# lenskit/csr

Measured on AMD Instinct MI355X. Metric: spmv_gflops, higher is better.
Workload: dtype f64

## Files before the change

### csr_amd/csrc/acc_groups.h

```cpp
#pragma once
#include <algorithm>
#include <cstdint>
#include <numeric>
#include <vector>

namespace csrk {
namespace accgroups {

constexpr int MAX_GROUPS = 3;
constexpr int XCDS = 8;

struct Deal {
    std::vector<std::vector<int32_t>> groups;
    std::vector<int32_t> first;
};

inline Deal deal_rows(const int64_t *lens, int32_t n, int G, int32_t cap)
{
    Deal d;
    d.first.push_back(0);
    if (n <= 0) return d;
    if (cap < 1) cap = 1;
    if (G < 1) G = 1;
    if (G > MAX_GROUPS) G = MAX_GROUPS;
// ... 24 lines not shown
}

constexpr int64_t TILE_ENTRIES = 512;
constexpr int64_t MIN_SEG_TILES = 48;
inline int choose_groups(const int64_t *lens, int32_t n, int g_max, int32_t cap, int64_t floor_len, int64_t nb, int32_t cus)
{
    if (cap < 1) cap = 1;
    if (g_max > MAX_GROUPS) g_max = MAX_GROUPS;
    if (g_max < 2 || n <= cap) return 1;
    std::vector<int64_t> sl;
    for (int32_t i = 0; i < n; i++)
        if (lens[i] >= floor_len) sl.push_back(lens[i]);
    for (int g = g_max; g > 1; g--) {
        const int64_t k = std::min<int64_t>((int64_t)sl.size(), (int64_t)g * cap);
        if (k <= (int64_t)(g - 1) * cap) continue;
        if (k < (int64_t)sl.size()) std::nth_element(sl.begin(), sl.begin() + k, sl.end(), [](int64_t a, int64_t b) { return a > b; });
        int64_t entries = 0;
        for (int64_t i = 0; i < k; i++) entries += sl[(size_t)i];
        if (entries / TILE_ENTRIES >= MIN_SEG_TILES * ((int64_t)g * nb + cus)) return g;
    }
    return 1;
}

inline int32_t group_wgs(int32_t cus, int gb, int g)
{
    const int32_t n = cus / gb + (g < cus % gb ? 1 : 0);
    return n < 1 ? 1 : n;
}

inline std::vector<uint32_t> place_wgs(const int32_t *n_wg, int gb)
{
    int64_t total = 0;
    int32_t w_max = 0;
    for (int g = 0; g < gb; g++) {
        total += n_wg[g];
        w_max = std::max(w_max, n_wg[g]);
    }
    std::vector<uint32_t> map((size_t)total, ~0u);
    int64_t fill[XCDS], room[XCDS];
    for (int c = 0; c < XCDS; c++) {
        fill[c] = 0;
        room[c] = total / XCDS + (c < total % XCDS ? 1 : 0);
    }
    std::vector<uint32_t> late;
    for (int32_t w = 0; w < w_max; w++)
        for (int g = 0; g < gb; g++) {
// ... 17 lines not shown
```

### csr_amd/csrc/fix56.h

```cpp
#pragma once
#include <cstdint>
#include <cstring>

#if defined(__HIPCC__)
#define FIX56_HD __host__ __device__ __forceinline__
#else
#define FIX56_HD inline
#endif

namespace csrk {
namespace fix56 {

constexpr int TILE = 512;
constexpr int LO_BYTES = TILE * 4, MID_BYTES = TILE * 2, HI_BYTES = TILE;
constexpr int MID_OFF = LO_BYTES, HI_OFF = LO_BYTES + MID_BYTES;
constexpr int TILE_BYTES = LO_BYTES + MID_BYTES + HI_BYTES;
constexpr uint64_t MANT_MASK = (1ull << 52) - 1;
constexpr uint32_t W_MANT = 0x000fffffu, W_SIGN = 0x00800000u;

struct Packed {
    unsigned char b[7];
};
static_assert(sizeof(Packed) * TILE == TILE_BYTES, "a tile of Packed entries is the three planes");

// ... 69 lines not shown
FIX56_HD double decode(uint32_t lo, uint32_t w, uint32_t ebits, double magic)
{
    const double d = double_of((w & W_MANT) | ebits, lo) - magic;
    return double_of((uint32_t)(bits_of(d) >> 32) ^ ((w & W_SIGN) << 8), (uint32_t)bits_of(d));
}
FIX56_HD uint32_t ebits_of(int32_t g) { return (uint32_t)(1075 + g) << 20; }
FIX56_HD double magic_of(int32_t g) { return double_of(ebits_of(g), 0u); }

FIX56_HD int lo_slot(int e) { return ((e & 7) >> 2) * 256 + (e >> 3) * 4 + (e & 3); }

FIX56_HD void put(unsigned char *tile, int e, uint64_t p)
{
    ((uint32_t *)tile)[lo_slot(e)] = lo_of(p);
    ((uint16_t *)(tile + MID_OFF))[e] = mid_of(p);
    tile[HI_OFF + e] = hi_of(p);
}
FIX56_HD double get(const unsigned char *tile, int e, int32_t g)
{
    const uint32_t lo = ((const uint32_t *)tile)[lo_slot(e)];
    const uint32_t w = (uint32_t)((const uint16_t *)(tile + MID_OFF))[e] | (uint32_t)tile[HI_OFF + e] << 16;
    return decode(lo, w, ebits_of(g), magic_of(g));
}

}
}
```

### csr_amd/csrc/spmv.hip

```cpp
#include "spmv_plan.h"

#include <algorithm>
#include <ctime>

namespace csrk {
template <bool R32>
__device__ __forceinline__ double spmv_prod(double a, double x)
{
    const double t = a * x;
    return R32 ? (double)(float)t : t;
}

void free_spmv_plan(SpmvPlan *p) { delete p; }

void spmv_plan_bytes_by_part(const SpmvPlan *p, int64_t out[5])
{
    for (int i = 0; i < 5; i++) out[i] = 0;
    auto add = [&](int part, std::initializer_list<const DevBuf *> bufs) {
        for (const DevBuf *b : bufs) out[part] += (int64_t)b->bytes;
    };
    for (const AccPanel *ap : p->acc) add(0, {&ap->row_list, &ap->vals, &ap->idx, &ap->tile_row0, &ap->segs, &ap->wg_seg, &ap->partial, &ap->z, &ap->wg_map});
    const Panel &t = p->tier1;
    add(1, {&t.row_list, &t.rp, &t.ci, &t.vs, &t.tile, &t.group, &t.carry_row, &t.carry_val, &t.y, &t.crp, &t.cidx});
    const LightStream *l = &p->ls;
// ... 462 lines not shown
                        v[u] = *((const F64x2 *)(x + w0) + tid + u * PT);
                    } else {
                        const f32x2_t t = *((const F32x2 *)(x + w0) + tid + u * PT);
                        v[u].x = (double)t.x;
                        v[u].y = (double)t.y;
                    }
                }
#pragma unroll
                for (int u = 0; u < WL; u++) ((f64x2_t *)s_x)[tid + u * PT] = v[u];
            } else {
                for (int k = tid; k < wlen; k += PT) s_x[k] = (double)x[w0 + k];
            }
        }
        __syncthreads();

        const int nt = sg.ntiles;
        AccVals<SV> v, vn;
        u32x4_t ix, ixn;
        int32_t tr0 = 0, tr0n = 0;
        int t = wv;
        const int64_t pstep = (int64_t)A.n_wg;
        if (t < nt) {
            const u32x4_t *ip = (const u32x4_t *)(pidx + (sg.ptile0 + t * pstep) * ACC_TILE);
            v.load(pvals + (sg.ptile0 + t * pstep) * ACC_TILE, lane);
            ix = __builtin_nontemporal_load(ip + lane);
            tr0 = tile_row0[sg.tile0 + t];
        }
        for (; t < nt; t += NW) {
            const bool more = t + NW < nt;
            if (more) {
                const u32x4_t *ip = (const u32x4_t *)(pidx + (sg.ptile0 + (t + NW) * pstep) * ACC_TILE);
                vn.load(pvals + (sg.ptile0 + (t + NW) * pstep) * ACC_TILE, lane);
                ixn = __builtin_nontemporal_load(ip + lane);
                tr0n = tile_row0[sg.tile0 + t + NW];
            }
            const uint32_t e[ACC_K] = {ix.x & 0xffffu, ix.x >> 16, ix.y & 0xffffu, ix.y >> 16,
                                       ix.z & 0xffffu, ix.z >> 16, ix.w & 0xffffu, ix.w >> 16};
            double a[ACC_K];
            v.get(a, fx_g);
            double xv[ACC_K];
#pragma unroll
            for (int j = 0; j < ACC_K; j++) xv[j] = s_x[e[j] & ACC_COL_MASK];
            int rw[ACC_K];
            {
                int lsum = 0;
#pragma unroll
                for (int j = 0; j < ACC_K; j++) lsum += (int)(e[j] >> ACC_ROW_SHIFT);
                int run = tr0 + wave_exscan_i32(lsum, lane);
#pragma unroll
                for (int j = 0; j < ACC_K; j++) {
                    run += (int)(e[j] >> ACC_ROW_SHIFT);
                    rw[j] = run;
                }
            }
            const int hr = rw[0];
            int cur = hr;
            double acc = 0.0, hs = 0.0;
            bool nb = false;
#pragma unroll
            for (int j = 0; j < ACC_K; j++) {
                const int r = rw[j];
                if (r != cur) {
// ... 535 lines not shown
{
    for (const void *f : {(const void *)spmv_acc_kernel<ACC_CB, ACC_THREADS>, (const void *)spmv_lstream_kernel<LS_PLAIN>,
                          (const void *)spmv_lstream_kernel<LS_RND>, (const void *)spmv_lstream_kernel<LS_PLAIN, true>,
                          (const void *)spmv_lstream_kernel<LS_RND, true>, (const void *)spmv_acc_kernel<ACC_CB, ACC_THREADS, true>,
                          (const void *)spmv_lstream_kernel<LS_PLAIN, false, true>, (const void *)spmv_lstream_kernel<LS_RND, false, true>,
                          (const void *)spmv_lstream_kernel<LS_PLAIN, true, true>, (const void *)spmv_lstream_kernel<LS_RND, true, true>,
                          (const void *)spmv_acc_kernel<ACC_CB, ACC_THREADS, false, float>,
                          (const void *)spmv_acc_kernel<ACC_CB, ACC_THREADS, true, float>,
                          (const void *)spmv_lstream_kernel<LS_PLAIN, false, false, float>, (const void *)spmv_lstream_kernel<LS_RND, false, false, float>,
                          (const void *)spmv_lstream_kernel<LS_PLAIN, true, false, float>, (const void *)spmv_lstream_kernel<LS_RND, true, false, float>,
                          (const void *)spmv_lstream_kernel<LS_PLAIN, false, true, float>, (const void *)spmv_lstream_kernel<LS_RND, false, true, float>,
                          (const void *)spmv_lstream_kernel<LS_PLAIN, true, true, float>, (const void *)spmv_lstream_kernel<LS_RND, true, true, float>,
                          (const void *)spmv_lstream_kernel<LS_RND24>, (const void *)spmv_lstream_kernel<LS_RND24, true>,
                          (const void *)spmv_lstream_kernel<LS_RND24, false, true>, (const void *)spmv_lstream_kernel<LS_RND24, true, true>,
                          (const void *)spmv_lstream_kernel<LS_RND24, false, false, float>, (const void *)spmv_lstream_kernel<LS_RND24, true, false, float>,
                          (const void *)spmv_lstream_kernel<LS_RND24, false, true, float>, (const void *)spmv_lstream_kernel<LS_RND24, true, true, float>,
                          (const void *)spmv_acc_kernel<ACC_CB, ACC_THREADS, false, double, float>,
                          (const void *)spmv_acc_kernel<ACC_CB, ACC_THREADS, true, double, float>,
                          (const void *)spmv_acc_kernel<ACC_CB, ACC_THREADS, false, float, float>,
                          (const void *)spmv_acc_kernel<ACC_CB, ACC_THREADS, true, float, float>,
                          (const void *)spmv_acc_kernel<ACC_CB, ACC_THREADS, false, fix56::Packed>,
                          (const void *)spmv_acc_kernel<ACC_CB, ACC_THREADS, true, fix56::Packed>,
                          (const void *)spmv_acc_kernel<ACC_CB, ACC_THREADS, false, fix56::Packed, float>,
                          (const void *)spmv_acc_kernel<ACC_CB, ACC_THREADS, true, fix56::Packed, float>})
        CSRK_HIP(hipFuncSetAttribute(f, hipFuncAttributeMaxDynamicSharedMemorySize, (int)(160 * 1024)));
    CSRK_HIP(hipFuncSetAttribute((const void *)ls_stage_kernel<double>, hipFuncAttributeMaxDynamicSharedMemorySize, (int)(LS_STAGE_WMAX * 8)));
    CSRK_HIP(hipFuncSetAttribute((const void *)ls_stage_kernel<float>, hipFuncAttributeMaxDynamicSharedMemorySize, (int)(LS_STAGE_WMAX * 8)));
    return CSRK_OK;
}

static int get_plan_locked(Matrix *m, hipStream_t s, SpmvPlan **out, bool launching)
{
    if (launching) m->spmv_calls++;
    const char *env = getenv("CSRK_SPMV_HEAVY_SPLIT"), *env_hot = getenv("CSRK_SPMV_HOT"), *env_ls = getenv("CSRK_SPMV_STREAM");
    const bool eager = (env && env[0] == '1') || (env_hot && env_hot[0] == '1') || (env_ls && env_ls[0] == '1') || !launching;
    const bool want_split = eager || m->spmv_calls >= 2;
    if (m->spmv_plan && !m->spmv_plan->split_considered && want_split && m->spmv_plan->algo == CSRK_SPMV_MERGE &&
        !m->spmv_plan->profiling) {
        if (hipDeviceSynchronize() != hipSuccess) {
            set_error("device synchronisation failed: %s", hipGetErrorString(hipGetLastError()));
            return CSRK_ERR_HIP;
        }
        free_spmv_plan(m->spmv_plan);
        m->spmv_plan = nullptr;
    }
    if (!m->spmv_plan) {
        SpmvPlan *p = new (std::nothrow) SpmvPlan();
// ... 92 lines not shown
        }
        bool t0_rides = false;
        if (do_heavy && p->n_heavy && !p->acc.empty()) {
            KernelTimer kh(p, s, 1);
            for (size_t a0 = 0; a0 < p->acc.size(); a0 += (size_t)p->acc[a0]->launch_groups) {
                AccPanel *ap = p->acc[a0];
                const int gb = ap->launch_groups;
                if (gb < 1 || gb > accgroups::MAX_GROUPS || a0 + (size_t)gb > p->acc.size()) {
                    set_error("internal: tier 0's groups and launches disagree");
                    return CSRK_ERR_INVALID;
                }
                AccLaunchArgs L = {};
                size_t lds = 0;
                for (int g = 0; g < gb; g++) {
                    const AccPanel *aq = p->acc[a0 + (size_t)g];
                    L.g[g] = {aq->vals.p, aq->idx.as<uint16_t>(), aq->tile_row0.as<int32_t>(), aq->segs.as<AccSeg>(),
                              aq->wg_seg.as<int32_t>(), aq->partial.as<double>(), aq->nrow, aq->n_wg, aq->fx_g, 0};
                    lds = aq->lds > lds ? aq->lds : lds;
                }
                L.wg_map = gb > 1 ? ap->wg_map.as<uint32_t>() : nullptr;
                const unsigned n_blocks = (unsigned)(gb > 1 ? ap->launch_wgs : ap->n_wg);
#define ACC_LAUNCH(SV) spmv_acc_kernel<ACC_CB, ACC_THREADS, R32, SV, XT><<<n_blocks, ACC_THREADS, lds, s>>>(L, d_x, m->ncols)
                if (ap->f32) ACC_LAUNCH(float);
                else if (ap->fix56) ACC_LAUNCH(fix56::Packed);
                else ACC_LAUNCH(double);
#undef ACC_LAUNCH
                CSRK_LAUNCH_CHECK();
            }
            kh.stop();
        }
        if (do_heavy && p->n_heavy && p->tier1.on) {
            Panel *pn = &p->tier1;
            KernelTimer kh(p, s, 2);
#define PANEL_ARGS(PP)                                                                                              \
    pn->rp.as<PP>(), pn->ci.as<int32_t>(), pn->vs.as<double>(), d_x, m->ncols, pn->y.as<double>(),                    \
        pn->tile.as<PanelTile>(), pn->group.as<PanelGroup>(), pn->rows, pn->carry_row.as<int32_t>(),                  \
        pn->carry_val.as<double>(), pn->nnz, pn->cb, rider
            PanelRider rider = {};
            rider.first = pn->groups;
            for (int q = 0; q < accgroups::MAX_GROUPS; q++) rider.start[q] = INT32_MAX;
            int64_t rider_wgs = 0;
            if (PANEL_T1 / WAVE == 4 && do_heavy && !p->acc.empty() && (size_t)p->acc[0]->launch_groups == p->acc.size() &&
                p->acc.size() <= (size_t)accgroups::MAX_GROUPS && p->acc[0]->z.p) {
                for (size_t q = 0; q < p->acc.size(); q++) {
                    AccPanel *ap = p->acc[q];
                    rider.partial[q] = ap->partial.as<double>();
// ... 501 lines not shown
```

### csr_amd/csrc/spmv_plan.h

```cpp
#pragma once
#include "common.h"
#include "wave.h"
#include "fix56.h"
#include "acc_groups.h"

#include <vector>

namespace csrk {

template <int VT> struct ValLoad;
template <> struct ValLoad<CSRK_VAL_F64> {
    static __device__ __forceinline__ double at(const void *v, int64_t k) { return ((const double *)v)[k]; }
};
template <> struct ValLoad<CSRK_VAL_F32> {
    static __device__ __forceinline__ double at(const void *v, int64_t k) { return (double)((const float *)v)[k]; }
};
template <> struct ValLoad<CSRK_VAL_NONE> {
    static __device__ __forceinline__ double at(const void *, int64_t) { return 1.0; }
};

__device__ __forceinline__ double wave_sum(double v)
{
#pragma unroll
    for (int off = WAVE / 2; off > 0; off >>= 1) v += __shfl_down(v, off, WAVE);
    return v;
}

__device__ __forceinline__ double ordered_sum(const double *p, int s, int e)
// ... 18 lines not shown
    DevBuf row_list;
    DevBuf rp, ci, vs, tile, group, carry_row, carry_val, y;
    int32_t ncs = 0;
    DevBuf crp, cidx;
};

struct AccSeg {
    int64_t tile0;
    int64_t ptile0;
    int32_t ntiles;
    int32_t blk;
};

struct AccPanel {
    int32_t nrow = 0, nb = 0, n_wg = 0;
    int32_t launch_groups = 1, launch_wgs = 0;
    DevBuf wg_map;
    int64_t tiles = 0, nnz = 0, n_segs = 0;
    size_t lds = 0;
    DevBuf row_list, vals, idx, tile_row0, segs, wg_seg, partial;
    DevBuf z;
    bool f32 = false;
    bool fix56 = false;
    int32_t fx_g = 0;
};

struct LightStream {
    bool on = false;
    int64_t n_tiles = 0;
    int32_t n_runs = 0, n_out = 0;
    unsigned grid = 0;
    DevBuf vals, idx, rowids, tile_base, carry_row, carry_val;
    bool idx24 = false;
    bool f32 = false;
    bool dense = false;
    int64_t n_cold = 0;
    int32_t n_stage_blk = 0, stage_w = 0;
    DevBuf xg, a_col, a_dst, blk_start;
    int32_t stage_tiles = 0;
    int32_t n_rounds = 0, max_wg_rounds = 0;
    DevBuf round_start, round_tile0, wg_round0;
};

struct SpmvPlan {
    int algo = CSRK_SPMV_MERGE;
    int tile_items = 0;
// ... 197 lines not shown
    __device__ __forceinline__ void load(const fix56::Packed *tile, int lane)
    {
        const unsigned char *tp = (const unsigned char *)tile;
#pragma unroll
        for (int q = 0; q < 2; q++) lo[q] = __builtin_nontemporal_load((const u32x4_t *)tp + q * WAVE + lane);
        mid = __builtin_nontemporal_load((const u32x4_t *)(tp + fix56::MID_OFF) + lane);
        hi = __builtin_nontemporal_load((const u32x2_t *)(tp + fix56::HI_OFF) + lane);
    }
    __device__ __forceinline__ void get(double (&a)[ACC_K], int32_t g) const
    {
        const uint32_t l[ACC_K] = {lo[0].x, lo[0].y, lo[0].z, lo[0].w, lo[1].x, lo[1].y, lo[1].z, lo[1].w};
        const uint32_t m[4] = {mid.x, mid.y, mid.z, mid.w}, h[2] = {hi.x, hi.y};
        const uint32_t ebits = fix56::ebits_of(g);
        const double magic = fix56::magic_of(g);
#pragma unroll
        for (int j = 0; j < ACC_K; j++) {
            const uint32_t w = __builtin_amdgcn_perm(h[j >> 2], m[j >> 1],
                                                     0x0c000000u | ((4u + (j & 3)) << 16) | ((2u * (j & 1) + 1u) << 8) | (2u * (j & 1)));
            a[j] = fix56::decode(l[j], w, ebits, magic);
        }
    }
};

#ifndef CSRK_LS_THREADS
#define CSRK_LS_THREADS 512
#endif
constexpr int LS_THREADS = CSRK_LS_THREADS;
#ifndef CSRK_LS_HOT_LDS
#define CSRK_LS_HOT_LDS 15360
#endif
constexpr int LS_HOT_LDS = CSRK_LS_HOT_LDS;
#ifndef CSRK_LS_RND_CAP
#define CSRK_LS_RND_CAP 8192
#endif
constexpr int LS_RND_CAP = CSRK_LS_RND_CAP, LS_RND_MAXTILES = 128;
constexpr int LS_RND_HOT = (160 * 1024 - (CSRK_LS_THREADS / 64) * (512 + 2) * 8) / 8 - LS_RND_CAP;
constexpr int LS_RID = 4;
#ifndef CSRK_LS_SEQ
#define CSRK_LS_SEQ 3
#endif
constexpr int LS_SEQ = CSRK_LS_SEQ;
constexpr uint32_t LS_HOT_BIT = 1u << 31, LS_START_BIT = 1u << 30, LS_COL_MASK = (1u << 30) - 1;
constexpr uint32_t LS_PAD = LS_COL_MASK;
#ifndef CSRK_LS_IDX24
#define CSRK_LS_IDX24 1
#endif
// ... 23 lines not shown
```

### csr_amd/csrc/spmv_plan.hip

```cpp
#include "spmv_plan.h"

#include <algorithm>
#include <cstring>
#include <ctime>
#include <type_traits>

namespace csrk {
struct PlanTrace {
    bool on;
    double t0;
    static double now()
    {
        timespec ts;
        clock_gettime(CLOCK_MONOTONIC, &ts);
        return ts.tv_sec * 1e3 + ts.tv_nsec * 1e-6;
    }
    PlanTrace() : on(getenv("CSRK_PLAN_TRACE") != nullptr), t0(0.0)
    {
        if (on) {
            (void)hipDeviceSynchronize();
            t0 = now();
        }
    }
    void lap(const char *what)
// ... 510 lines not shown
                                                       const int32_t *__restrict__ rows, int32_t *__restrict__ out)
{
    const int32_t row = rows[blockIdx.x];
    const int64_t k1 = (int64_t)rp[row + 1];
    fix56::Range r;
    for (int64_t k = (int64_t)rp[row] + blockIdx.y * 256 + threadIdx.x; k < k1; k += (int64_t)gridDim.y * 256) fix56::fold(r, vs[k]);
#pragma unroll
    for (int off = WAVE / 2; off > 0; off >>= 1) {
        fix56::Range o;
        o.bad = __shfl_xor(r.bad, off, WAVE);
        o.lo = __shfl_xor(r.lo, off, WAVE);
        o.hi = __shfl_xor(r.hi, off, WAVE);
        fix56::merge(r, o);
    }
    if ((threadIdx.x & (WAVE - 1)) == 0) {
        const volatile int32_t *seen = out;
        if (r.bad && !seen[0]) atomicOr(out, 1);
        if (r.lo < seen[1]) atomicMin(out + 1, r.lo);
        if (r.hi > seen[2]) atomicMax(out + 2, r.hi);
    }
}

template <class SV, bool VERIFY>
__device__ __forceinline__ void acc_put(SV *__restrict__ pvals, int64_t pt, int el, double v, int32_t fx_g,
                                        int32_t *__restrict__ mismatch)
{
    if constexpr (!std::is_same<SV, fix56::Packed>::value) {
        pvals[pt * ACC_TILE + acc_slot_of<SV>(el)] = (SV)v;
    } else if constexpr (!VERIFY) {
        fix56::put((unsigned char *)(pvals + pt * ACC_TILE), el, fix56::encode(v, fx_g));
    } else {
        AccVals<SV> t;
        t.load(pvals + pt * ACC_TILE, el >> 3);
        double a[ACC_K];
        t.get(a, fx_g);
        double d = a[0];
#pragma unroll
        for (int j = 1; j < ACC_K; j++) d = (el & 7) == j ? a[j] : d;
        if (fix56::bits_of(d) != fix56::bits_of(v)) *mismatch = 1;
    }
}

template <class P, int VT, class SV, bool VERIFY = false>
__global__ __launch_bounds__(256) void acc_fill_kernel(const P *__restrict__ rp, const int32_t *__restrict__ ci,
                                                      const void *__restrict__ vs, const int32_t *__restrict__ heavy_row,
                                                      int32_t n_heavy, int32_t n_blocks, int32_t cb,
                                                      const int64_t *__restrict__ off, const int64_t *__restrict__ blk_tile0,
                                                      const int32_t *__restrict__ pstart, const int32_t *__restrict__ gap,
                                                      SV *__restrict__ pvals, uint16_t *__restrict__ pidx,
                                                      int32_t *__restrict__ tile_row0, const int64_t *__restrict__ wg_t0,
                                                      int32_t n_wg, int32_t waves_per_block, int32_t fx_g,
                                                      int32_t *__restrict__ mismatch)
{
// ... 17 lines not shown
    const int32_t start = wave_exscan_i32(n_all, lane);
    const int32_t total = __builtin_amdgcn_readlane(start + n_all, WAVE - 1);
    if (total == 0) return;
    const int64_t L0 = blk_tile0[b] * ACC_TILE + (__shfl(off_i, 0, WAVE) - off[(int64_t)b * n_heavy]);
    int32_t *starts = s_start[wv];
    starts[lane] = start;
    __builtin_amdgcn_wave_barrier();
    for (int32_t d0 = 0; d0 < total; d0 += WAVE) {
        const int32_t d = d0 + lane;
        const bool in = d < total;
        int p = 0;
#pragma unroll
        for (int step = WAVE / 2; step; step >>= 1)
            if (in && starts[p + step] <= d) p += step;
        const int32_t at = d - __shfl(start, p, WAVE);
        const int32_t npad_p = __shfl(npad, p, WAVE), g_p = __shfl(g, p, WAVE);
        const int64_t lo_p = __shfl(lo, p, WAVE);
        if (!in) continue;
        const int64_t L = L0 + d;
        const int64_t t = L / ACC_TILE;
        const int el = (int)(L % ACC_TILE);
        const int64_t pt = acc_phys_tile(t, wg_t0, n_wg);
        if (at < npad_p) {
            acc_put<SV, VERIFY>(pvals, pt, el, 0.0, fx_g, mismatch);
            if (VERIFY) continue;
            pidx[pt * ACC_TILE + el] = (uint16_t)((uint32_t)cb | ((el ? (uint32_t)ACC_MAXSTEP : 0u) << ACC_ROW_SHIFT));
            if (el == 0) tile_row0[t] = c0 + p - g_p + ACC_MAXSTEP * (at + 1);
        } else {
            const int64_t k = lo_p + (at - npad_p);
            const uint32_t step_in = at == npad_p ? (uint32_t)(g_p - ACC_MAXSTEP * npad_p) : 0u;
            acc_put<SV, VERIFY>(pvals, pt, el, ValLoad<VT>::at(vs, k), fx_g, mismatch);
            if (VERIFY) continue;
            pidx[pt * ACC_TILE + el] = (uint16_t)((uint32_t)(ci[k] - b * cb) | ((el ? step_in : 0u) << ACC_ROW_SHIFT));
            if (el == 0) tile_row0[t] = c0 + p;
        }
    }
}

template <class SV, bool VERIFY = false>
__global__ __launch_bounds__(256) void acc_pad_kernel(const int64_t *__restrict__ off, int32_t n_heavy, int32_t n_blocks,
                                                     const int64_t *__restrict__ blk_tile0, SV *__restrict__ pvals,
                                                     uint16_t *__restrict__ pidx, const int64_t *__restrict__ wg_t0, int32_t n_wg,
                                                     int32_t fx_g, int32_t *__restrict__ mismatch)
{
    const int32_t b = blockIdx.x;
    if (b >= n_blocks) return;
    const int64_t cnt = off[(int64_t)(b + 1) * n_heavy] - off[(int64_t)b * n_heavy];
    const int64_t L0 = blk_tile0[b] * ACC_TILE + cnt, L1 = blk_tile0[b + 1] * ACC_TILE;
    for (int64_t L = L0 + threadIdx.x; L < L1; L += blockDim.x) {
        const int64_t pt = acc_phys_tile(L / ACC_TILE, wg_t0, n_wg);
        const int el = (int)(L % ACC_TILE);
        acc_put<SV, VERIFY>(pvals, pt, el, 0.0, fx_g, mismatch);
        if (!VERIFY) pidx[pt * ACC_TILE + el] = (uint16_t)ACC_CB;
    }
}


template <class P>
__device__ __forceinline__ int32_t ls_row_of(const P *__restrict__ rpv, int32_t nrows, int64_t L)
{
    int32_t lo = 0, hi = nrows - 1;
    while (lo < hi) {
        const int32_t mid = lo + ((hi - lo) >> 1);
        if ((int64_t)rpv[mid + 1] > L)
            hi = mid;
        else
            lo = mid + 1;
    }
    return lo;
}

template <class P>
__global__ void ls_tilerow_kernel(const P *__restrict__ rpv, int32_t nrows, int64_t n_ent, int64_t n_tiles, int32_t *__restrict__ tile_row)
{
    const int64_t t = (int64_t)blockIdx.x * blockDim.x + threadIdx.x;
    if (t > n_tiles) return;
// ... 211 lines not shown
    pn->groups = (int64_t)groups.size();
    CSRK_TRY(pn->group.alloc(groups.size() * sizeof(PanelGroup)));
    CSRK_TRY(stage_h2d(pn->group.p, groups.data(), groups.size() * sizeof(PanelGroup), s));
    CSRK_TRY(pn->carry_row.alloc((size_t)n_tiles * 4));
    CSRK_TRY(pn->carry_val.alloc((size_t)n_tiles * 8));
    CSRK_TRY(pn->y.alloc((size_t)(pairs + (int64_t)ncs * n) * 8));
    if (ncs) {
        std::vector<double> neg0((size_t)ncs * n, -0.0);
        CSRK_TRY(stage_h2d(pn->y.as<double>() + pairs, neg0.data(), neg0.size() * 8, s));
    }
    pn->ncs = ncs;
    CSRK_HIP(hipStreamSynchronize(s));
    tr.lap("  tier 1: groups, carries (host)");
    pn->on = true;
    pn->cb = cb;
    pn->nb = nb;
    pn->nrow = n;
    pn->rows = pairs;
    pn->tiles = n_tiles;
    pn->nnz = nnz_rows;
    return CSRK_OK;
}

template <class P, int VT>
static int build_acc_panel(Matrix *m, AccPanel *ap, const int32_t *rows, const int64_t *lens, int32_t n, int64_t nnz_rows,
                           hipStream_t s, int32_t wg_want = 0, bool allow_fix56 = true)
{
    ap->fix56 = false;
    ap->fx_g = 0;
    const P *rp = (const P *)m->d_rowptrs;
    const int32_t nb = (int32_t)ceil_div(m->ncols > 0 ? m->ncols : 1, ACC_CB);
    PlanTrace tr;
    const int64_t pairs = (int64_t)n * nb;
    CSRK_TRY(ap->row_list.alloc((size_t)n * 4));
    CSRK_TRY(stage_h2d(ap->row_list.p, rows, (size_t)n * 4, s));
    DevBuf off, bends, pstart, d_trow, d_tpiece;
    CSRK_TRY(off.alloc((size_t)(pairs + 1) * 8));
    std::vector<int32_t> trow, tpiece;
    for (int32_t c = 0; c < n; c++)
        for (int64_t pc = 0; pc * ACC_PIECE < lens[c]; pc++) {
            trow.push_back(c);
            tpiece.push_back((int32_t)pc);
        }
    const int64_t n_tasks = (int64_t)trow.size();
    CSRK_TRY(pstart.alloc((size_t)(pairs + n) * 4));
    CSRK_TRY(d_trow.alloc((size_t)(n_tasks ? n_tasks : 1) * 4));
    CSRK_TRY(d_tpiece.alloc((size_t)(n_tasks ? n_tasks : 1) * 4));
    CSRK_TRY(stage_h2d(d_trow.p, trow.data(), (size_t)n_tasks * 4, s));
    CSRK_TRY(stage_h2d(d_tpiece.p, tpiece.data(), (size_t)n_tasks * 4, s));
    acc_pairstart_kernel<P><<<(unsigned)(ceil_div(ceil_div(n_tasks * WAVE, 256), 8) * 8), 256, 0, s>>>(
        rp, m->d_colinds, ap->row_list.as<int32_t>(), n, nb, ACC_CB, d_trow.as<int32_t>(), d_tpiece.as<int32_t>(), n_tasks,
// ... 14 lines not shown
    CSRK_TRY(stage_d2h(be.data(), bends.p, (size_t)(nb + 1) * 8, s));
    CSRK_HIP(hipStreamSynchronize(s));
    t0[0] = 0;
    for (int32_t b = 0; b < nb; b++) t0[b + 1] = t0[b] + ceil_div(be[b + 1] - be[b], ACC_TILE);
    const int64_t n_tiles = t0[nb];
    CSRK_TRY(stage_h2d(bends.p, t0.data(), (size_t)(nb + 1) * 8, s));
    tr.lap("  tier 0: counts, gaps, scan");
    int cus = 0;
    CSRK_HIP(hipDeviceGetAttribute(&cus, hipDeviceAttributeMultiprocessorCount, m->device));
    int64_t n_wg = wg_want > 0 ? wg_want : cus > 0 ? cus : 256;
    if (n_wg > n_tiles) n_wg = n_tiles;
    if (n_wg < 1) n_wg = 1;
    std::vector<int64_t> wg_t0((size_t)n_wg + 1);
    int64_t share_max = 0;
    for (int64_t w = 0; w <= n_wg; w++) wg_t0[(size_t)w] = n_tiles * w / n_wg;
    for (int64_t w = 0; w < n_wg; w++) share_max = std::max(share_max, wg_t0[(size_t)w + 1] - wg_t0[(size_t)w]);
    const int64_t n_phys = share_max * n_wg;
    DevBuf d_wg_t0;
    CSRK_TRY(d_wg_t0.alloc((size_t)(n_wg + 1) * 8));
    CSRK_TRY(stage_h2d(d_wg_t0.p, wg_t0.data(), (size_t)(n_wg + 1) * 8, s));
    ap->f32 = VT == CSRK_VAL_F32;
    DevBuf fx;
    CSRK_TRY(fx.alloc(16));
    if (VT == CSRK_VAL_F64 && n > 0 && allow_fix56) {
        const char *env = getenv("CSRK_SPMV_FIX56");
        if (!(env && env[0] == '0')) {
            int32_t h[4] = {0, INT32_MAX, INT32_MIN, 0};
            CSRK_TRY(stage_h2d(fx.p, h, sizeof h, s));
            acc_range_kernel<P><<<dim3((unsigned)n, 16), 256, 0, s>>>(rp, (const double *)m->d_values, ap->row_list.as<int32_t>(),
                                                                     fx.as<int32_t>());
            CSRK_LAUNCH_CHECK();
            CSRK_TRY(stage_d2h(h, fx.p, sizeof h, s));
            CSRK_HIP(hipStreamSynchronize(s));
            fix56::Range r;
            r.bad = h[0];
            r.lo = h[1];
            r.hi = h[2];
            ap->fix56 = fix56::packable(r, ap->fx_g);
            tr.lap("  tier 0: value grid test");
        }
    }
    CSRK_TRY(ap->idx.alloc((size_t)n_phys * ACC_TILE * 2));
    CSRK_TRY(ap->tile_row0.alloc((size_t)(n_tiles ? n_tiles : 1) * 4));
    const int32_t fill_waves = (int32_t)ceil_div(n, WAVE);
#define ACC_FILL(SV, VERIFY)                                                                                           \
    do {                                                                                                               \
        acc_fill_kernel<P, VT, SV, VERIFY><<<(unsigned)ceil_div((int64_t)nb * fill_waves * WAVE, 256), 256, 0, s>>>(   \
            rp, m->d_colinds, m->d_values, ap->row_list.as<int32_t>(), n, nb, ACC_CB, off.as<int64_t>(),               \
            bends.as<int64_t>(), pstart.as<int32_t>(), gap.as<int32_t>(), ap->vals.as<SV>(), ap->idx.as<uint16_t>(),   \
            ap->tile_row0.as<int32_t>(), d_wg_t0.as<int64_t>(), (int32_t)n_wg, fill_waves, ap->fx_g,                   \
            fx.as<int32_t>() + 3);                                                                                     \
        CSRK_LAUNCH_CHECK();                                                                                           \
        acc_pad_kernel<SV, VERIFY><<<(unsigned)nb, 256, 0, s>>>(off.as<int64_t>(), n, nb, bends.as<int64_t>(),         \
                                                                ap->vals.as<SV>(), ap->idx.as<uint16_t>(),             \
                                                                d_wg_t0.as<int64_t>(), (int32_t)n_wg, ap->fx_g,        \
                                                                fx.as<int32_t>() + 3);                                 \
        CSRK_LAUNCH_CHECK();                                                                                           \
    } while (0)
    if (ap->fix56) {
        CSRK_TRY(ap->vals.alloc((size_t)n_phys * fix56::TILE_BYTES));
        ACC_FILL(fix56::Packed, false);
        tr.lap("  tier 0: fill (fix56)");
        int32_t mismatch = 1;
        ACC_FILL(fix56::Packed, true);
        CSRK_TRY(stage_d2h(&mismatch, fx.as<int32_t>() + 3, 4, s));
        CSRK_HIP(hipStreamSynchronize(s));
        tr.lap("  tier 0: verify (fix56)");
        if (mismatch) {
            ap->fix56 = false;
            ap->fx_g = 0;
        }
    }
    if (!ap->fix56) {
        CSRK_TRY(ap->vals.alloc((size_t)n_phys * ACC_TILE * (ap->f32 ? 4 : 8)));
        if (ap->f32) ACC_FILL(float, false);
        else ACC_FILL(double, false);
        tr.lap("  tier 0: fill");
    }
#undef ACC_FILL
    std::vector<AccSeg> segs;
    std::vector<int32_t> wg_seg((size_t)n_wg + 1);
    int32_t b = 0;
    for (int64_t w = 0; w < n_wg; w++) {
        wg_seg[(size_t)w] = (int32_t)segs.size();
        int64_t t = wg_t0[(size_t)w];
        const int64_t t_end = wg_t0[(size_t)w + 1];
        while (t < t_end) {
            while (t0[b + 1] <= t) b++;
            int64_t e = t_end < t0[b + 1] ? t_end : t0[b + 1];
            if (e - t > ACC_SEG_TILES) e = t + ACC_SEG_TILES;
            AccSeg sg;
            sg.tile0 = t;
// ... 3 lines not shown
            segs.push_back(sg);
            t = e;
        }
    }
    wg_seg[(size_t)n_wg] = (int32_t)segs.size();
    CSRK_TRY(ap->segs.alloc(segs.size() * sizeof(AccSeg)));
    CSRK_TRY(ap->wg_seg.alloc(wg_seg.size() * 4));
    CSRK_TRY(stage_h2d(ap->segs.p, segs.data(), segs.size() * sizeof(AccSeg), s));
    CSRK_TRY(stage_h2d(ap->wg_seg.p, wg_seg.data(), wg_seg.size() * 4, s));
    CSRK_TRY(ap->partial.alloc((size_t)n_wg * n * 8));
    CSRK_TRY(ap->z.alloc((size_t)n * 8));
    ap->lds = (size_t)(ACC_CB + 2) * 8 + (size_t)((n + 1) & ~1) * 8 + (size_t)ACC_SEG_TILES * 12;
    CSRK_TRY(spmv_kernel_attributes());
    CSRK_HIP(hipStreamSynchronize(s));
    ap->nrow = n;
    ap->nb = nb;
    ap->n_wg = (int32_t)n_wg;
    ap->tiles = n_tiles;
    ap->nnz = nnz_rows;
    ap->n_segs = (int64_t)segs.size();
    if (tr.on)
        fprintf(stderr, "[csrk plan]   tier 0 group: rows %d entries %lld workgroups %lld tiles %lld, %.1f per segment%s\n", n,
                (long long)nnz_rows, (long long)n_wg, (long long)n_tiles, segs.empty() ? 0.0 : (double)n_tiles / (double)segs.size(),
                ap->fix56 ? " (fix56)" : "");
    tr.lap("  tier 0: segments");
    return CSRK_OK;
}

static int acc_groups_knob()
{
    const char *e = getenv("CSRK_ACC_GROUPS");
    const int g = e ? atoi(e) : ACC_GROUPS_DEFAULT;
    return g < 1 ? 1 : g > accgroups::MAX_GROUPS ? accgroups::MAX_GROUPS : g;
}
static int32_t acc_group_rows_knob()
{
    const char *e = getenv("CSRK_ACC_GROUP_ROWS");
    const int r = e ? atoi(e) : ACC_MAXROWS;
    return r < 1 || r > ACC_MAXROWS ? ACC_MAXROWS : r;
}


template <class P>
static int build_heavy_split(Matrix *m, SpmvPlan *p, hipStream_t s, bool allow_tier1 = true)
{
    p->n_heavy = 0;
    const char *env = getenv("CSRK_SPMV_HEAVY_SPLIT");
    if (env && env[0] == '0') return CSRK_OK;
    HEAVY_MIN = 2048;
// ... 117 lines not shown
    p->t0_rows = std::move(r0);
    p->t0_lens = std::move(len0);
    p->t1_rows = std::move(r1);
    p->t1_nnz = nnz1;
    tr.lap("  split: host lists");
    return CSRK_OK;
}

template <class P, int VT>
static int build_acc_groups(Matrix *m, SpmvPlan *p, hipStream_t s)
{
    const std::vector<int32_t> &r0 = p->t0_rows;
    const std::vector<int64_t> &len0 = p->t0_lens;
    if (r0.empty()) return CSRK_OK;
    const accgroups::Deal deal = accgroups::deal_rows(len0.data(), (int32_t)r0.size(), p->acc_groups, acc_group_rows_knob());
    int cus = 0;
    CSRK_HIP(hipDeviceGetAttribute(&cus, hipDeviceAttributeMultiprocessorCount, m->device));
    if (cus <= 0) cus = 256;
    std::vector<int32_t> rows;
    std::vector<int64_t> lens;
    for (size_t j = 0; j + 1 < deal.first.size(); j++) {
        const int k0 = deal.first[j], gb = deal.first[j + 1] - k0;
        const size_t a0 = p->acc.size();
        auto build = [&](int g, bool allow_fix56) -> int {
            const std::vector<int32_t> &pos = deal.groups[(size_t)(k0 + g)];
            rows.resize(pos.size());
            lens.resize(pos.size());
            int64_t gn = 0;
            for (size_t i = 0; i < pos.size(); i++) {
                rows[i] = r0[(size_t)pos[i]];
                lens[i] = len0[(size_t)pos[i]];
                gn += lens[i];
            }
            return build_acc_panel<P, VT>(m, p->acc[a0 + (size_t)g], rows.data(), lens.data(), (int32_t)pos.size(), gn, s,
                                          gb > 1 ? accgroups::group_wgs(cus, gb, g) : 0, allow_fix56);
        };
        bool any_raw = false;
        for (int g = 0; g < gb; g++) {
            AccPanel *ap = new (std::nothrow) AccPanel();
            CSRK_REQUIRE(ap, "out of host memory");
            p->acc.push_back(ap);
            CSRK_TRY(build(g, true));
            any_raw = any_raw || !ap->fix56;
        }
        AccPanel *head = p->acc[a0];
        if (gb == 1) continue;
        for (int g = 0; g < gb; g++)
            if (any_raw && p->acc[a0 + (size_t)g]->fix56) CSRK_TRY(build(g, false));
        int32_t n_wg[accgroups::MAX_GROUPS];
        for (int g = 0; g < gb; g++) {
            n_wg[g] = p->acc[a0 + (size_t)g]->n_wg;
            p->acc[a0 + (size_t)g]->launch_groups = 0;
        }
        const std::vector<uint32_t> map = accgroups::place_wgs(n_wg, gb);
        head->launch_groups = gb;
        head->launch_wgs = (int32_t)map.size();
        CSRK_TRY(head->wg_map.alloc(map.size() * 4));
        CSRK_TRY(stage_h2d(head->wg_map.p, map.data(), map.size() * 4, s));
        CSRK_HIP(hipStreamSynchronize(s));
    }
    return CSRK_OK;
}

template <class P>
static int build_tiers(Matrix *m, SpmvPlan *p, hipStream_t s)
{
    if (!p->n_heavy) return CSRK_OK;
    const std::vector<int32_t> &r1 = p->t1_rows;
    const int64_t nnz1 = p->t1_nnz;
#define BUILD(VT)                                                                                                  \
    do {                                                                                                           \
// ... 645 lines not shown
```

Baseline: 818.1.

## Add 52-bit nibble-packed tile format storing sign and top bits in index word

Adds a 'nib' variant of the fix56 tile encoding that shrinks the high plane from a byte to a nibble per entry. The sign bit moves into the spare bit of the 16-bit column/step index word, cutting value bytes per nonzero from 7 to 6.5. It is chosen automatically when a launch has enough tiles per workgroup, and is meant to reduce HBM traffic in the bandwidth-bound f64 SpMV. In exchange it packs 12-bit columns, adds decode ALU work (perm, masks) and uses atomicOr during fill, and it only applies when values fit the 52-bit grid.

```diff
diff --git a/csr_amd/csrc/acc_groups.h b/csr_amd/csrc/acc_groups.h
--- a/csr_amd/csrc/acc_groups.h
+++ b/csr_amd/csrc/acc_groups.h
@@ -70,6 +70,14 @@
     return 1;
 }
 
+constexpr int64_t NIB_MIN_WG_TILES = 16;
+inline bool choose_nib(int knob, int64_t launch_entries, int32_t launch_wgs)
+{
+    if (knob >= 0) return knob != 0;
+    if (launch_wgs < 1) launch_wgs = 1;
+    return launch_entries >= 0 && launch_entries / TILE_ENTRIES >= NIB_MIN_WG_TILES * (int64_t)launch_wgs;
+}
+
 inline int32_t group_wgs(int32_t cus, int gb, int g)
 {
     const int32_t n = cus / gb + (g < cus % gb ? 1 : 0);
diff --git a/csr_amd/csrc/fix56.h b/csr_amd/csrc/fix56.h
--- a/csr_amd/csrc/fix56.h
+++ b/csr_amd/csrc/fix56.h
@@ -115,5 +115,69 @@
     return decode(lo, w, ebits_of(g), magic_of(g));
 }
 
+namespace nib {
+
+constexpr int LO_BYTES = TILE * 4, MID_BYTES = TILE * 2, HI_BYTES = TILE / 2;
+constexpr int MID_OFF = LO_BYTES, HI_OFF = LO_BYTES + MID_BYTES;
+constexpr int TILE_BYTES = LO_BYTES + MID_BYTES + HI_BYTES;
+constexpr int COL_BITS = 12, STEP_SHIFT = 12;
+constexpr uint32_t COL_MASK = (1u << COL_BITS) - 1, STEP_MASK = 7u, SIGN = 1u << 15;
+constexpr uint32_t PAD_COL = 1u << COL_BITS;
+constexpr uint64_t PAD_CODE = 1ull << 55;
+
+struct Bytes {
+    unsigned char b;
+};
+
+FIX56_HD uint16_t index_word(uint64_t p, uint32_t col, uint32_t step)
+{
+    const bool pad = p == PAD_CODE;
+    return (uint16_t)((pad ? 0u : col & COL_MASK) | (step & STEP_MASK) << STEP_SHIFT | (uint32_t)(p >> 55) << 15);
+}
+FIX56_HD int hi_word(int e) { return e >> 3; }
+FIX56_HD int hi_shift(int e) { return (e & 7) * 4; }
+FIX56_HD uint32_t hi_of(uint64_t p) { return (uint32_t)(p >> 48) & 0xfu; }
+
+FIX56_HD double join(uint32_t hi, uint32_t lo)
+{
+    const uint32_t t[2] = {lo, hi};
+    double v;
+    memcpy(&v, t, 8);
+    return v;
+}
+FIX56_HD uint32_t high_of(double v)
+{
+    uint32_t t[2];
+    memcpy(t, &v, 8);
+    return t[1];
+}
+
+FIX56_HD double entry(uint32_t lo, uint32_t hi, uint32_t word, double magic, uint32_t &col, uint32_t &step)
+{
+    const double d = join(hi, lo) - magic;
+    const double a = join(high_of(d) | ((word << 16) & 0x80000000u), (uint32_t)bits_of(d));
+    col = bits_of(a) == 1ull << 63 ? PAD_COL : word & COL_MASK;
+    step = (word >> STEP_SHIFT) & STEP_MASK;
+    return a;
+}
+
+FIX56_HD void put(unsigned char *tile, uint16_t *idx, int e, uint64_t p, uint32_t col, uint32_t step)
+{
+    ((uint32_t *)tile)[lo_slot(e)] = lo_of(p);
+    ((uint16_t *)(tile + MID_OFF))[e] = mid_of(p);
+    uint32_t *h = (uint32_t *)(tile + HI_OFF) + hi_word(e);
+    *h = (*h & ~(0xfu << hi_shift(e))) | hi_of(p) << hi_shift(e);
+    idx[e] = index_word(p, col, step);
+}
+FIX56_HD double get(const unsigned char *tile, const uint16_t *idx, int e, int32_t g, uint32_t &col, uint32_t &step)
+{
+    const uint32_t lo = ((const uint32_t *)tile)[lo_slot(e)];
+    const uint32_t nibble = (((const uint32_t *)(tile + HI_OFF))[hi_word(e)] >> hi_shift(e)) & 0xfu;
+    const uint32_t w = (uint32_t)((const uint16_t *)(tile + MID_OFF))[e] | nibble << 16;
+    return entry(lo, w | ebits_of(g), idx[e], magic_of(g), col, step);
+}
+
+}
+
 }
 }
diff --git a/csr_amd/csrc/spmv.hip b/csr_amd/csrc/spmv.hip
--- a/csr_amd/csrc/spmv.hip
+++ b/csr_amd/csrc/spmv.hip
@@ -508,7 +508,7 @@
         const int64_t pstep = (int64_t)A.n_wg;
         if (t < nt) {
             const u32x4_t *ip = (const u32x4_t *)(pidx + (sg.ptile0 + t * pstep) * ACC_TILE);
-            v.load(pvals + (sg.ptile0 + t * pstep) * ACC_TILE, lane);
+            v.load(acc_tile_at(pvals, sg.ptile0 + t * pstep), lane);
             ix = __builtin_nontemporal_load(ip + lane);
             tr0 = tile_row0[sg.tile0 + t];
         }
@@ -516,14 +516,15 @@
             const bool more = t + NW < nt;
             if (more) {
                 const u32x4_t *ip = (const u32x4_t *)(pidx + (sg.ptile0 + (t + NW) * pstep) * ACC_TILE);
-                vn.load(pvals + (sg.ptile0 + (t + NW) * pstep) * ACC_TILE, lane);
+                vn.load(acc_tile_at(pvals, sg.ptile0 + (t + NW) * pstep), lane);
                 ixn = __builtin_nontemporal_load(ip + lane);
                 tr0n = tile_row0[sg.tile0 + t + NW];
             }
-            const uint32_t e[ACC_K] = {ix.x & 0xffffu, ix.x >> 16, ix.y & 0xffffu, ix.y >> 16,
-                                       ix.z & 0xffffu, ix.z >> 16, ix.w & 0xffffu, ix.w >> 16};
+            uint32_t e[ACC_K] = {ix.x & 0xffffu, ix.x >> 16, ix.y & 0xffffu, ix.y >> 16,
+                                 ix.z & 0xffffu, ix.z >> 16, ix.w & 0xffffu, ix.w >> 16};
             double a[ACC_K];
-            v.get(a, fx_g);
+            if constexpr (std::is_same<SV, fix56::nib::Bytes>::value) v.get(a, fx_g, e);
+            else v.get(a, fx_g);
             double xv[ACC_K];
 #pragma unroll
             for (int j = 0; j < ACC_K; j++) xv[j] = s_x[e[j] & ACC_COL_MASK];
@@ -1105,7 +1106,11 @@
                           (const void *)spmv_acc_kernel<ACC_CB, ACC_THREADS, false, fix56::Packed>,
                           (const void *)spmv_acc_kernel<ACC_CB, ACC_THREADS, true, fix56::Packed>,
                           (const void *)spmv_acc_kernel<ACC_CB, ACC_THREADS, false, fix56::Packed, float>,
-                          (const void *)spmv_acc_kernel<ACC_CB, ACC_THREADS, true, fix56::Packed, float>})
+                          (const void *)spmv_acc_kernel<ACC_CB, ACC_THREADS, true, fix56::Packed, float>,
+                          (const void *)spmv_acc_kernel<ACC_CB, ACC_THREADS, false, fix56::nib::Bytes>,
+                          (const void *)spmv_acc_kernel<ACC_CB, ACC_THREADS, true, fix56::nib::Bytes>,
+                          (const void *)spmv_acc_kernel<ACC_CB, ACC_THREADS, false, fix56::nib::Bytes, float>,
+                          (const void *)spmv_acc_kernel<ACC_CB, ACC_THREADS, true, fix56::nib::Bytes, float>})
         CSRK_HIP(hipFuncSetAttribute(f, hipFuncAttributeMaxDynamicSharedMemorySize, (int)(160 * 1024)));
     CSRK_HIP(hipFuncSetAttribute((const void *)ls_stage_kernel<double>, hipFuncAttributeMaxDynamicSharedMemorySize, (int)(LS_STAGE_WMAX * 8)));
     CSRK_HIP(hipFuncSetAttribute((const void *)ls_stage_kernel<float>, hipFuncAttributeMaxDynamicSharedMemorySize, (int)(LS_STAGE_WMAX * 8)));
@@ -1244,6 +1249,7 @@
                 const unsigned n_blocks = (unsigned)(gb > 1 ? ap->launch_wgs : ap->n_wg);
 #define ACC_LAUNCH(SV) spmv_acc_kernel<ACC_CB, ACC_THREADS, R32, SV, XT><<<n_blocks, ACC_THREADS, lds, s>>>(L, d_x, m->ncols)
                 if (ap->f32) ACC_LAUNCH(float);
+                else if (ap->nib) ACC_LAUNCH(fix56::nib::Bytes);
                 else if (ap->fix56) ACC_LAUNCH(fix56::Packed);
                 else ACC_LAUNCH(double);
 #undef ACC_LAUNCH
diff --git a/csr_amd/csrc/spmv_plan.h b/csr_amd/csrc/spmv_plan.h
--- a/csr_amd/csrc/spmv_plan.h
+++ b/csr_amd/csrc/spmv_plan.h
@@ -4,6 +4,7 @@
 #include "fix56.h"
 #include "acc_groups.h"
 
+#include <type_traits>
 #include <vector>
 
 namespace csrk {
@@ -68,6 +69,7 @@
     DevBuf z;
     bool f32 = false;
     bool fix56 = false;
+    bool nib = false;
     int32_t fx_g = 0;
 };
 
@@ -311,6 +313,40 @@
     }
 };
 
+static_assert(fix56::nib::PAD_COL == (uint32_t)ACC_CB, "a padding entry of a nib tile reads the window's zero slot");
+template <> struct AccVals<fix56::nib::Bytes> {
+    u32x4_t lo[2], mid;
+    uint32_t hi;
+    __device__ __forceinline__ void load(const fix56::nib::Bytes *tile, int lane)
+    {
+        const unsigned char *tp = (const unsigned char *)tile;
+#pragma unroll
+        for (int q = 0; q < 2; q++) lo[q] = __builtin_nontemporal_load((const u32x4_t *)tp + q * WAVE + lane);
+        mid = __builtin_nontemporal_load((const u32x4_t *)(tp + fix56::nib::MID_OFF) + lane);
+        hi = __builtin_nontemporal_load((const uint32_t *)(tp + fix56::nib::HI_OFF) + lane);
+    }
+    __device__ __forceinline__ void get(double (&a)[ACC_K], int32_t g, uint32_t (&e)[ACC_K]) const
+    {
+        const uint32_t l[ACC_K] = {lo[0].x, lo[0].y, lo[0].z, lo[0].w, lo[1].x, lo[1].y, lo[1].z, lo[1].w};
+        const uint32_t m[4] = {mid.x, mid.y, mid.z, mid.w};
+        const uint32_t ebits = fix56::ebits_of(g);
+        const double magic = fix56::magic_of(g);
+#pragma unroll
+        for (int j = 0; j < ACC_K; j++) {
+            const uint32_t top = ((hi >> (4 * j)) & 0xfu) | ebits >> 16;
+            const uint32_t w = __builtin_amdgcn_perm(top, m[j >> 1], 0x05040000u | ((2u * (j & 1) + 1u) << 8) | (2u * (j & 1)));
+            uint32_t col, step;
+            a[j] = fix56::nib::entry(l[j], w, e[j], magic, col, step);
+            e[j] = col | step << ACC_ROW_SHIFT;
+        }
+    }
+};
+template <class SV> __host__ __device__ __forceinline__ SV *acc_tile_at(SV *vals, int64_t t)
+{
+    if constexpr (sizeof(SV) == 1) return vals + t * fix56::nib::TILE_BYTES;
+    else return vals + t * ACC_TILE;
+}
+
 #ifndef CSRK_LS_THREADS
 #define CSRK_LS_THREADS 512
 #endif
diff --git a/csr_amd/csrc/spmv_plan.hip b/csr_amd/csrc/spmv_plan.hip
--- a/csr_amd/csrc/spmv_plan.hip
+++ b/csr_amd/csrc/spmv_plan.hip
@@ -556,13 +556,42 @@
 }
 
 template <class SV, bool VERIFY>
-__device__ __forceinline__ void acc_put(SV *__restrict__ pvals, int64_t pt, int el, double v, int32_t fx_g,
-                                        int32_t *__restrict__ mismatch)
-{
-    if constexpr (!std::is_same<SV, fix56::Packed>::value) {
+__device__ __forceinline__ void acc_put(SV *__restrict__ pvals, uint16_t *__restrict__ pidx, int64_t pt, int el, double v,
+                                        uint32_t col, uint32_t step, int32_t fx_g, int32_t *__restrict__ mismatch)
+{
+    if constexpr (std::is_same<SV, fix56::nib::Bytes>::value) {
+        namespace nib = fix56::nib;
+        unsigned char *tile = (unsigned char *)acc_tile_at(pvals, pt);
+        const bool pad = col == (uint32_t)ACC_CB;
+        if constexpr (!VERIFY) {
+            const uint64_t p = pad ? nib::PAD_CODE : fix56::encode(v, fx_g);
+            ((uint32_t *)tile)[fix56::lo_slot(el)] = fix56::lo_of(p);
+            ((uint16_t *)(tile + nib::MID_OFF))[el] = fix56::mid_of(p);
+            if (nib::hi_of(p)) atomicOr((uint32_t *)(tile + nib::HI_OFF) + nib::hi_word(el), nib::hi_of(p) << nib::hi_shift(el));
+            pidx[pt * ACC_TILE + el] = nib::index_word(p, col, step);
+        } else {
+            AccVals<SV> t;
+            t.load((const SV *)tile, el >> 3);
+            const u32x4_t ix = *((const u32x4_t *)(pidx + pt * ACC_TILE) + (el >> 3));
+            uint32_t e[ACC_K] = {ix.x & 0xffffu, ix.x >> 16, ix.y & 0xffffu, ix.y >> 16,
+                                 ix.z & 0xffffu, ix.z >> 16, ix.w & 0xffffu, ix.w >> 16};
+            double a[ACC_K];
+            t.get(a, fx_g, e);
+            double d = a[0];
+            uint32_t w = e[0];
+#pragma unroll
+            for (int j = 1; j < ACC_K; j++) {
+                d = (el & 7) == j ? a[j] : d;
+                w = (el & 7) == j ? e[j] : w;
+            }
+            if (fix56::bits_of(d) != (pad ? 1ull << 63 : fix56::bits_of(v)) || w != (col | step << ACC_ROW_SHIFT)) *mismatch = 1;
+        }
+    } else if constexpr (!std::is_same<SV, fix56::Packed>::value) {
         pvals[pt * ACC_TILE + acc_slot_of<SV>(el)] = (SV)v;
+        pidx[pt * ACC_TILE + el] = (uint16_t)(col | step << ACC_ROW_SHIFT);
     } else if constexpr (!VERIFY) {
         fix56::put((unsigned char *)(pvals + pt * ACC_TILE), el, fix56::encode(v, fx_g));
+        pidx[pt * ACC_TILE + el] = (uint16_t)(col | step << ACC_ROW_SHIFT);
     } else {
         AccVals<SV> t;
         t.load(pvals + pt * ACC_TILE, el >> 3);
@@ -626,16 +655,15 @@
         const int el = (int)(L % ACC_TILE);
         const int64_t pt = acc_phys_tile(t, wg_t0, n_wg);
         if (at < npad_p) {
-            acc_put<SV, VERIFY>(pvals, pt, el, 0.0, fx_g, mismatch);
+            acc_put<SV, VERIFY>(pvals, pidx, pt, el, 0.0, (uint32_t)cb, el ? (uint32_t)ACC_MAXSTEP : 0u, fx_g, mismatch);
             if (VERIFY) continue;
-            pidx[pt * ACC_TILE + el] = (uint16_t)((uint32_t)cb | ((el ? (uint32_t)ACC_MAXSTEP : 0u) << ACC_ROW_SHIFT));
             if (el == 0) tile_row0[t] = c0 + p - g_p + ACC_MAXSTEP * (at + 1);
         } else {
             const int64_t k = lo_p + (at - npad_p);
             const uint32_t step_in = at == npad_p ? (uint32_t)(g_p - ACC_MAXSTEP * npad_p) : 0u;
-            acc_put<SV, VERIFY>(pvals, pt, el, ValLoad<VT>::at(vs, k), fx_g, mismatch);
+            acc_put<SV, VERIFY>(pvals, pidx, pt, el, ValLoad<VT>::at(vs, k), (uint32_t)(ci[k] - b * cb), el ? step_in : 0u, fx_g,
+                                mismatch);
             if (VERIFY) continue;
-            pidx[pt * ACC_TILE + el] = (uint16_t)((uint32_t)(ci[k] - b * cb) | ((el ? step_in : 0u) << ACC_ROW_SHIFT));
             if (el == 0) tile_row0[t] = c0 + p;
         }
     }
@@ -654,8 +682,7 @@
     for (int64_t L = L0 + threadIdx.x; L < L1; L += blockDim.x) {
         const int64_t pt = acc_phys_tile(L / ACC_TILE, wg_t0, n_wg);
         const int el = (int)(L % ACC_TILE);
-        acc_put<SV, VERIFY>(pvals, pt, el, 0.0, fx_g, mismatch);
-        if (!VERIFY) pidx[pt * ACC_TILE + el] = (uint16_t)ACC_CB;
+        acc_put<SV, VERIFY>(pvals, pidx, pt, el, 0.0, (uint32_t)ACC_CB, 0u, fx_g, mismatch);
     }
 }
 
@@ -913,11 +940,13 @@
     return CSRK_OK;
 }
 
+enum { ACC_FORM_RAW = 0, ACC_FORM_FIX56 = 1, ACC_FORM_NIB = 2 };
 template <class P, int VT>
 static int build_acc_panel(Matrix *m, AccPanel *ap, const int32_t *rows, const int64_t *lens, int32_t n, int64_t nnz_rows,
-                           hipStream_t s, int32_t wg_want = 0, bool allow_fix56 = true)
+                           hipStream_t s, int32_t wg_want = 0, int form = ACC_FORM_FIX56)
 {
     ap->fix56 = false;
+    ap->nib = false;
     ap->fx_g = 0;
     const P *rp = (const P *)m->d_rowptrs;
     const int32_t nb = (int32_t)ceil_div(m->ncols > 0 ? m->ncols : 1, ACC_CB);
@@ -978,7 +1007,7 @@
     ap->f32 = VT == CSRK_VAL_F32;
     DevBuf fx;
     CSRK_TRY(fx.alloc(16));
-    if (VT == CSRK_VAL_F64 && n > 0 && allow_fix56) {
+    if (VT == CSRK_VAL_F64 && n > 0 && form != ACC_FORM_RAW) {
         const char *env = getenv("CSRK_SPMV_FIX56");
         if (!(env && env[0] == '0')) {
             int32_t h[4] = {0, INT32_MAX, INT32_MIN, 0};
@@ -993,6 +1022,7 @@
             r.lo = h[1];
             r.hi = h[2];
             ap->fix56 = fix56::packable(r, ap->fx_g);
+            ap->nib = ap->fix56 && form == ACC_FORM_NIB;
             tr.lap("  tier 0: value grid test");
         }
     }
@@ -1014,16 +1044,24 @@
         CSRK_LAUNCH_CHECK();                                                                                           \
     } while (0)
     if (ap->fix56) {
-        CSRK_TRY(ap->vals.alloc((size_t)n_phys * fix56::TILE_BYTES));
-        ACC_FILL(fix56::Packed, false);
-        tr.lap("  tier 0: fill (fix56)");
         int32_t mismatch = 1;
-        ACC_FILL(fix56::Packed, true);
+        if (ap->nib) {
+            CSRK_TRY(ap->vals.alloc((size_t)n_phys * fix56::nib::TILE_BYTES));
+            CSRK_HIP(hipMemsetAsync(ap->vals.p, 0, (size_t)n_phys * fix56::nib::TILE_BYTES, s));
+            ACC_FILL(fix56::nib::Bytes, false);
+            tr.lap("  tier 0: fill (nib)");
+            ACC_FILL(fix56::nib::Bytes, true);
+        } else {
+            CSRK_TRY(ap->vals.alloc((size_t)n_phys * fix56::TILE_BYTES));
+            ACC_FILL(fix56::Packed, false);
+            tr.lap("  tier 0: fill (fix56)");
+            ACC_FILL(fix56::Packed, true);
+        }
         CSRK_TRY(stage_d2h(&mismatch, fx.as<int32_t>() + 3, 4, s));
         CSRK_HIP(hipStreamSynchronize(s));
-        tr.lap("  tier 0: verify (fix56)");
+        tr.lap(ap->nib ? "  tier 0: verify (nib)" : "  tier 0: verify (fix56)");
         if (mismatch) {
-            ap->fix56 = false;
+            ap->fix56 = ap->nib = false;
             ap->fx_g = 0;
         }
     }
@@ -1073,9 +1111,16 @@
     if (tr.on)
         fprintf(stderr, "[csrk plan]   tier 0 group: rows %d entries %lld workgroups %lld tiles %lld, %.1f per segment%s\n", n,
                 (long long)nnz_rows, (long long)n_wg, (long long)n_tiles, segs.empty() ? 0.0 : (double)n_tiles / (double)segs.size(),
-                ap->fix56 ? " (fix56)" : "");
+                ap->nib ? " (nib)" : ap->fix56 ? " (fix56)" : ap->f32 ? " (float32)" : " (raw)");
     tr.lap("  tier 0: segments");
     return CSRK_OK;
+}
+
+static int acc_nib_knob()
+{
+    const char *env = getenv("CSRK_SPMV_NIB");
+    if (!env || !env[0]) return -1;
+    return env[0] == '0' ? 0 : 1;
 }
 
 static int acc_groups_knob()
@@ -1239,7 +1284,11 @@
     for (size_t j = 0; j + 1 < deal.first.size(); j++) {
         const int k0 = deal.first[j], gb = deal.first[j + 1] - k0;
         const size_t a0 = p->acc.size();
-        auto build = [&](int g, bool allow_fix56) -> int {
+        int64_t launch_entries = 0;
+        for (int g = 0; g < gb; g++)
+            for (int32_t pos : deal.groups[(size_t)(k0 + g)]) launch_entries += len0[(size_t)pos];
+        const int packed = accgroups::choose_nib(acc_nib_knob(), launch_entries, cus) ? ACC_FORM_NIB : ACC_FORM_FIX56;
+        auto build = [&](int g, int form) -> int {
             const std::vector<int32_t> &pos = deal.groups[(size_t)(k0 + g)];
             rows.resize(pos.size());
             lens.resize(pos.size());
@@ -1250,20 +1299,20 @@
                 gn += lens[i];
             }
             return build_acc_panel<P, VT>(m, p->acc[a0 + (size_t)g], rows.data(), lens.data(), (int32_t)pos.size(), gn, s,
-                                          gb > 1 ? accgroups::group_wgs(cus, gb, g) : 0, allow_fix56);
+                                          gb > 1 ? accgroups::group_wgs(cus, gb, g) : 0, form);
         };
         bool any_raw = false;
         for (int g = 0; g < gb; g++) {
             AccPanel *ap = new (std::nothrow) AccPanel();
             CSRK_REQUIRE(ap, "out of host memory");
             p->acc.push_back(ap);
-            CSRK_TRY(build(g, true));
+            CSRK_TRY(build(g, packed));
             any_raw = any_raw || !ap->fix56;
         }
         AccPanel *head = p->acc[a0];
         if (gb == 1) continue;
         for (int g = 0; g < gb; g++)
-            if (any_raw && p->acc[a0 + (size_t)g]->fix56) CSRK_TRY(build(g, false));
+            if (any_raw && p->acc[a0 + (size_t)g]->fix56) CSRK_TRY(build(g, ACC_FORM_RAW));
         int32_t n_wg[accgroups::MAX_GROUPS];
         for (int g = 0; g < gb; g++) {
             n_wg[g] = p->acc[a0 + (size_t)g]->n_wg;
```

Measured after the change: 839.3 (median of 6 runs). 1.03x the previous value.
